# google-deepmind/meltingpot

Measured on NVIDIA H100. Metric: env_steps_per_sec, higher is better.
Workload: dtype u8

## Files before the change

include/mp_engine.h:

```cpp
#ifndef MP_ENGINE_H_
#define MP_ENGINE_H_

#include <stddef.h>
#include <stdint.h>

#ifdef __cplusplus
extern "C" {
#endif

typedef struct mp_engine* mp_handle;

enum {
  MP_OK = 0,
  MP_E_INVALID = -1,
  MP_E_UNSUPPORTED = -2,
  MP_E_CUDA = -3,
  MP_E_NO_DEVICE = -4
};

enum {
  MP_FLAG_RENDER_WORLD = 1u << 0,
  MP_FLAG_RENDER_PLAYERS = 1u << 1,
  MP_FLAG_DEFAULT = 3u,
  MP_FLAG_DEBUG_NO_COMPOSE = 1u << 4,
  MP_FLAG_DEBUG_NO_STORE = 1u << 5,
  MP_FLAG_DEBUG_REUSE_RECORDS = 1u << 6,
  MP_FLAG_DEBUG_NO_FENCE = 1u << 7,
  MP_FLAG_DEBUG_TOP_SPRITE_ONLY = 1u << 8,
  MP_FLAG_DEBUG_PLAIN_LANE_MAP = 1u << 9,
  MP_FLAG_DEBUG_SCATTER_LANE_MAP = 1u << 10,
  MP_FLAG_DEBUG_NO_PREMERGE = 1u << 11,
  MP_FLAG_LAYOUT_TEAMS_SHIFT = 16,
  MP_FLAG_LAYOUT_WARPS_SHIFT = 19,
  MP_FLAG_LAYOUT_WLOG_SHIFT = 24,
  MP_FLAG_LAYOUT_MASK = 0x3ffu << 16
};
#define MP_RENDER_LAYOUT(teams, warps, wlog) \
  (((uint32_t)(teams) << MP_FLAG_LAYOUT_TEAMS_SHIFT) | ((uint32_t)(warps) << MP_FLAG_LAYOUT_WARPS_SHIFT) | ((uint32_t)(wlog) << MP_FLAG_LAYOUT_WLOG_SHIFT))
#define MP_FLAGS_CREATE_ONLY (MP_FLAG_DEBUG_PLAIN_LANE_MAP | MP_FLAG_DEBUG_SCATTER_LANE_MAP | MP_FLAG_DEBUG_NO_PREMERGE | MP_FLAG_LAYOUT_MASK)

typedef struct mp_buffers {
  int32_t num_envs, num_players;
  int32_t rgb_h, rgb_w;
  int32_t world_h, world_w;
  int32_t num_actions;
  int32_t num_scalar_obs;
  uint8_t* rgb;
  uint8_t* world_rgb;
  double* reward;
  double* discount;
  int64_t* step_type;
  double* scalar_obs;
  int32_t* avatar_state;
  uint16_t* grid;
  int32_t grid_layers, grid_cells, grid_cells_padded;
  double* timestep_packed;
  int32_t* events;
  int32_t* event_count;
  int32_t max_events;
// ... 81 lines not shown
```

meltingpot_b200/csrc/engine.cu:

```cuda
#include <cuda_runtime.h>

#include <algorithm>
#include <cstdio>
#include <cstring>
#include <string>
#include <vector>

#include "../../include/mp_engine.h"
#include "../../include/mpb_format.h"
#include "common.cuh"
#include "family_load.h"
#include "render.cuh"
#include "step_clean_up.cuh"
#include "step_commons.cuh"
#include "step_territory.cuh"
#include "step_coins.cuh"
#include "step_mining.cuh"

namespace {

constexpr int kRenderSmemLimit = 227 * 1024 - 2560;
constexpr int kMaxAtlasSprites = 96;
#define MP_MAX_DEVICES 64
#define MP_EXCHANGE_HEADER 256
// ... 406 lines not shown
  for (int i = 0; i < n_total; ++i)
    for (int px = 0; px < 256; ++px) { const uint8_t a = img[(size_t)i * 1024 + px * 4 + 3]; if (a != 0 && a != 255) { binary_alpha[i] = 0; break; } }
  for (int i = 0; i < n_total; ++i) {
    bool bin = true;
    for (int v = 0; v <= T.P; ++v) bin = bin && binary_alpha[smap[(size_t)v * n_total + i]];
    bool invisible = true;
    for (int v = 0; v <= T.P && invisible; ++v) {
      const int t = smap[(size_t)v * n_total + i];
      for (int px = 0; px < 256 && invisible; ++px) invisible = img[(size_t)t * 1024 + px * 4 + 3] == 0;
    }
    sflags[i] = (uint8_t)((opq[i] ? 1 : 0) | (remapped[i] ? 2 : 0) | (bin ? 4 : 0) | (invisible ? 8 : 0));
  }
  E->host_pair = pair; E->host_sflags = sflags;
  E->black_sprite = -1;
  for (int i = 0; i < n_total && E->black_sprite < 0; ++i) {
    if (!opq[i] || remapped[i]) continue;
    bool black = true;
    for (int px = 0; px < 256 && black; ++px) { const uint8_t* q = &img[(size_t)i * 1024 + px * 4]; black = q[0] == 0 && q[1] == 0 && q[2] == 0; }
    if (black) E->black_sprite = i;
  }
  if ((rc = upload(E->allocs, smap, &T.sprite_map)) || (rc = upload(E->allocs, sflags, &T.sprite_opaque)) || (rc = upload(E->allocs, pair, &T.sprite_pair))) return rc;
  return MP_OK;
}

int build_plan(mp_engine* E) {
  const Tables& T = E->T;
  RenderPlan& R = E->R;
  R.view_w = T.view_l + T.view_r + 1; R.view_h = T.view_f + T.view_b + 1;
  R.player_bytes = R.view_w * R.view_h * 192;
  R.world_bytes = T.H * T.W * 192;
  R.grid_bytes = T.L * T.cells_pad * 2;
  R.n_total = E->n_total;
  R.atlas_bytes = R.n_total * 1024;
  R.rec_stride = (int)round_up(T.L + 1, 4);
  R.magic_view_h = (65536u + R.view_h - 1) / R.view_h;
  int off = 128;
  R.off_atlas = off; off += round_up(R.atlas_bytes, 128);
  R.off_pair = off; off += round_up(R.n_total * R.n_total, 128);
  R.off_map = off; off += round_up((T.P + 1) * R.n_total * 2, 128);
  R.off_team0 = off;
  const int f_teams = (E->flags >> MP_FLAG_LAYOUT_TEAMS_SHIFT) & 7, f_warps = (E->flags >> MP_FLAG_LAYOUT_WARPS_SHIFT) & 31,
            f_wlog = (E->flags >> MP_FLAG_LAYOUT_WLOG_SHIFT) & 3;
  const bool forced = (E->flags & MP_FLAG_LAYOUT_MASK) != 0;
  if (forced) {
    if (f_teams < 2 || f_teams > RENDER_MAX_TEAMS || f_warps < 4 || f_warps > TEAM_THREADS / 32 || f_wlog < 1 || f_wlog > 2)
      return fail(MP_E_INVALID, "render layout (%d teams, %d warps, wstrip_log2 %d) outside 2-%d / 4-%d / 1-2", f_teams, f_warps, f_wlog,
                  RENDER_MAX_TEAMS, TEAM_THREADS / 32);
    if (f_teams * f_warps > RENDER_MAX_THREADS / 32)
      return fail(MP_E_UNSUPPORTED, "render layout of %d teams x %d warps exceeds %d threads per CTA", f_teams, f_warps, RENDER_MAX_THREADS);
  }
  R.smem_bytes = 1 << 30;
  int need_forced = 0;
  double best = -1.0;
  for (int teams = 2; teams <= RENDER_MAX_TEAMS; ++teams)
    for (int warps = TEAM_THREADS / 32; warps >= 4; --warps) {
      if (teams * warps > RENDER_MAX_THREADS / 32) continue;
      if (forced && (teams != f_teams || warps != f_warps)) continue;
      for (int wlog = 2; wlog >= 1; --wlog) {
        if (forced && wlog != f_wlog) continue;
        const int stage = RENDER_SLOTS * round_up(std::max(R.view_w * 192, T.W * 24 * (1 << wlog)), 128);
        const int team_bytes = round_up(R.grid_bytes, 128) + round_up(T.cells * R.rec_stride * 2, 128) + warps * stage;
        const int total = R.off_team0 + teams * team_bytes;
        if (forced) need_forced = total;
        if (total > kRenderSmemLimit) continue;
        const double items = T.P * R.view_h + (8 >> wlog) * T.H, per_warp = items / warps;
        const double score = std::min(teams * warps, 18) * per_warp / (per_warp + 4.0) * (wlog == 2 ? 1.0 : 0.85) * (1.0 + 0.1 * teams);
        if (score > best + 1e-9) {
          best = score;
          R.n_teams = teams; R.team_threads = warps * 32; R.wstrip_log2 = wlog; R.stage_bytes = stage;
          R.toff_grid = 0; R.toff_rec = round_up(R.grid_bytes, 128);
          R.toff_stage = R.toff_rec + round_up(T.cells * R.rec_stride * 2, 128);
          R.team_stride = team_bytes; R.smem_bytes = total;
        }
      }
    }
  if (forced && R.smem_bytes > kRenderSmemLimit)
    return fail(MP_E_UNSUPPORTED, "render layout (%d teams, %d warps, wstrip_log2 %d) needs %d B of shared memory (> %d)", f_teams, f_warps,
                f_wlog, need_forced, kRenderSmemLimit);
  if (R.smem_bytes > kRenderSmemLimit) return fail(MP_E_UNSUPPORTED, "render kernel needs %d B of shared memory (> 227 KB)", R.smem_bytes);
  return MP_OK;
}

__global__ void k_debug_obs(Tables T, State S, int32_t* position, int32_t* orientation, int32_t* layer, int32_t* zap, int view_w, int view_h) {
  const int b = blockIdx.x, P = T.P;
  const int32_t* av = S.avatar + (size_t)b * P * 4;
  for (int p = threadIdx.x; p < P; p += blockDim.x) {
    if (position) { position[((size_t)b * P + p) * 2] = av[p * 4 + AV_X]; position[((size_t)b * P + p) * 2 + 1] = av[p * 4 + AV_Y]; }
    if (orientation) orientation[(size_t)b * P + p] = av[p * 4 + AV_ORIENT];
  }
  if (layer) {
    const int per_player = view_h * view_w * T.L;
    const uint16_t* grid = S.grid + (size_t)b * T.L * T.cells_pad;
    for (int i = threadIdx.x; i < P * per_player; i += blockDim.x) {
      const int p = i / per_player, r = i - p * per_player, l = r % T.L, c = r / T.L, vx = c % view_w, vy = c / view_w;
      int x = av[p * 4 + AV_X] - T.view_l + vx, y = av[p * 4 + AV_Y] - T.view_f + vy;
      int32_t v = -1;
      if (wrap_or_reject(T, x, y)) { const uint16_t g = grid[(size_t)l * T.cells_pad + y * T.W + x]; v = g ? ((g - 1) >> 2) + 1 : 0; }
      layer[(size_t)b * P * per_player + i] = v;
    }
  }
  if (zap) {
    for (int i = threadIdx.x; i < P * P; i += blockDim.x) zap[(size_t)b * P * P + i] = 0;
    __syncthreads();
    const int n = min(S.n_events[b], S.max_events);
// ... 535 lines not shown
  memcpy(&hd, host_src, sizeof(hd));
  if (memcmp(hd.magic, "MPS3", 4) != 0 || hd.version != 3u) return fail(MP_E_INVALID, "mp_state_load: not a snapshot (or one of an older engine)");
  if (hd.num_envs != (uint64_t)h->B || hd.payload_bytes != h->state_bytes || hd.n_spans != h->state_spans.size())
    return fail(MP_E_INVALID, "mp_state_load: snapshot of %llu envs / %llu bytes does not fit this engine (%d envs / %llu bytes)",
                (unsigned long long)hd.num_envs, (unsigned long long)hd.payload_bytes, h->B, (unsigned long long)h->state_bytes);
  if (nbytes != sizeof(SnapshotHeader) + hd.payload_bytes)
    return fail(MP_E_INVALID, "mp_state_load: buffer of %llu bytes, snapshot needs %llu (truncated?)", (unsigned long long)nbytes,
                (unsigned long long)(sizeof(SnapshotHeader) + hd.payload_bytes));
  if (hd.blob_hash != h->blob_hash) return fail(MP_E_INVALID, "mp_state_load: snapshot was taken from a different compiled substrate");
  if (hd.rng_key0 != h->S.seed) return fail(MP_E_INVALID, "mp_state_load: snapshot was taken with a different seed / env_index_base (key %llu, engine %llu)",
                                            (unsigned long long)hd.rng_key0, (unsigned long long)h->S.seed);
  DeviceGuard guard(h->device);
  cudaStream_t st = (cudaStream_t)stream;
  const uint8_t* src = static_cast<const uint8_t*>(host_src) + sizeof(hd);
  for (const auto& sp : h->state_spans) {
    CUDA_TRY(cudaMemcpyAsync(sp.first, src, sp.second, cudaMemcpyHostToDevice, st));
    src += sp.second;
  }
  int rc = launch_render(h, st);
  if (rc) return rc;
  CUDA_TRY(cudaStreamSynchronize(st));
  return MP_OK;
}

int mp_launch_count(mp_handle h, uint64_t* out) {
  if (!h || !out) return fail(MP_E_INVALID, "null argument");
  *out = h->launches;
  return MP_OK;
}

int mp_debug_render_plan(mp_handle h, int32_t out[MP_RENDER_PLAN_FIELDS]) {
  if (!h || !out) return fail(MP_E_INVALID, "mp_debug_render_plan: null argument");
  const RenderPlan& R = h->R;
  const int32_t v[MP_RENDER_PLAN_FIELDS] = {R.n_teams, R.team_threads, R.wstrip_log2, R.smem_bytes, R.n_total, R.rec_stride, R.stage_bytes,
                                            R.grid_bytes, h->lane_map_players, h->lane_map_world, h->inst_ncp, h->inst_ncw};
  memcpy(out, v, sizeof v);
  return MP_OK;
}

int mp_debug_render_tables(mp_handle h, int32_t* n_total, uint8_t* pair, uint8_t* flags) {
  if (!h) return fail(MP_E_INVALID, "null handle");
  if (n_total) *n_total = h->n_total;
  if (pair) memcpy(pair, h->host_pair.data(), h->host_pair.size());
  if (flags) memcpy(flags, h->host_sflags.data(), h->host_sflags.size());
  return MP_OK;
}

int mp_debug_observations(mp_handle h, int32_t* position, int32_t* orientation, int32_t* layer, int32_t* zap_matrix, void* stream) {
  if (!h) return fail(MP_E_INVALID, "null handle");
  DeviceGuard guard(h->device);
  k_debug_obs<<<h->B, 128, 0, (cudaStream_t)stream>>>(h->T, h->S, position, orientation, layer, zap_matrix, h->R.view_w, h->R.view_h);
  ++h->launches;
  CUDA_TRY(cudaGetLastError());
  return MP_OK;
}

int mp_debug_lane_map(int n_rows, int n_cells, int pitch_slots, int iters, int scattered, uint32_t out[32]) {
  if (!out || (n_rows != 8 && n_rows != 4 && n_rows != 2) || n_cells < 1 || n_cells > 62 || iters < 1 || iters > 5) return fail(MP_E_INVALID, "mp_debug_lane_map: bad arguments");
  if (!scattered) { if (n_cells > (32 / n_rows) * iters) return fail(MP_E_INVALID, "mp_debug_lane_map: too few turns"); make_lane_map_cells(n_rows, n_cells, pitch_slots, iters, out); return MP_OK; }
  if (!make_lane_map(n_rows, n_cells, pitch_slots, iters, out)) return fail(MP_E_UNSUPPORTED, "no conflict-free dealing for %d rows x %d cells in %d turns", n_rows, n_cells, iters);
  return MP_OK;
}

int mp_algorithmic_bytes(mp_handle h, uint64_t* per_env_step, uint64_t* render_per_env_step) {
  if (!h) return fail(MP_E_INVALID, "null handle");
  if (per_env_step) *per_env_step = h->algo_bytes;
  if (render_per_env_step) *render_per_env_step = h->render_bytes;
// ... 5 lines not shown
```

meltingpot_b200/csrc/render.cuh:

```cuda
#pragma once

#include <cstdio>

#include "common.cuh"

#define RENDER_MAX_TEAMS 4
#define RENDER_MAX_THREADS 1024
#ifndef TEAM_THREADS
#define TEAM_THREADS 512
#endif
#ifndef RENDER_SLOTS
#define RENDER_SLOTS 1
#endif

struct RenderPlan {
  int view_w, view_h;
  int player_bytes;
  int world_bytes;
  int grid_bytes;
  int atlas_bytes;
  int n_total;
  int rec_stride;
  uint32_t magic_view_h;
  int off_atlas, off_pair, off_map, off_team0, team_stride;
  int toff_grid, toff_rec, toff_stage;
  int wstrip_log2;
  int stage_bytes;
  int smem_bytes;
  int team_threads;
  int n_teams;
  int n_player_items, n_items;
  int prow_bytes, wrow_bytes;
  int pitem_bytes, witem_bytes;
  int h_oob, h_oov;
  int h_empty;
  uint32_t pmap[32], wmap[32];
};

__device__ __forceinline__ uint32_t smem_u32(const void* p) { return (uint32_t)__cvta_generic_to_shared(p); }

__device__ __forceinline__ void mbar_init(uint64_t* bar, int count) {
  asm volatile("mbarrier.init.shared::cta.b64 [%0], %1;" ::"r"(smem_u32(bar)), "r"(count));
}
__device__ __forceinline__ void mbar_expect_tx(uint64_t* bar, uint32_t bytes) {
  asm volatile("mbarrier.arrive.expect_tx.shared::cta.b64 _, [%0], %1;" ::"r"(smem_u32(bar)), "r"(bytes) : "memory");
}
__device__ __forceinline__ void mbar_wait(uint64_t* bar, uint32_t parity) {
  asm volatile(
      "{\n"
      ".reg .pred p;\n"
      "WAIT_%=:\n"
      "mbarrier.try_wait.parity.shared::cta.b64 p, [%0], %1;\n"
      "@p bra DONE_%=;\n"
      "bra WAIT_%=;\n"
      "DONE_%=:\n"
      "}\n" ::"r"(smem_u32(bar)), "r"(parity) : "memory");
}
__device__ __forceinline__ void bulk_load(void* dst_smem, const void* src_gmem, uint32_t bytes, uint64_t* bar) {
// ... 7 lines not shown
  return policy;
}
__device__ __forceinline__ void bulk_store(void* dst_gmem, const void* src_smem, uint32_t bytes, uint64_t policy) {
  asm volatile("cp.async.bulk.global.shared::cta.bulk_group.L2::cache_hint [%0], [%1], %2, %3;" ::"l"(dst_gmem), "r"(smem_u32(src_smem)),
               "r"(bytes), "l"(policy)
               : "memory");
  asm volatile("cp.async.bulk.commit_group;" ::: "memory");
}
template <int N>
__device__ __forceinline__ void bulk_wait_read() {
  asm volatile("cp.async.bulk.wait_group.read %0;" ::"n"(N) : "memory");
}
__device__ __forceinline__ void fence_async_smem() { asm volatile("fence.proxy.async.shared::cta;" ::: "memory"); }
__device__ __forceinline__ void group_sync(int bar_id, int threads) { asm volatile("bar.sync %0, %1;" ::"r"(bar_id), "r"(threads) : "memory"); }

__device__ __forceinline__ uint32_t blend_px(uint32_t dst, uint32_t src) {
  const uint32_t a = src >> 24;
  const uint32_t ia = 255u - a;
  uint32_t rb = (src & 0x00FF00FFu) * a + (dst & 0x00FF00FFu) * ia;
  uint32_t g = ((src >> 8) & 0xFFu) * a + ((dst >> 8) & 0xFFu) * ia;
  rb += 0x00010001u; rb += (rb >> 8) & 0x00FF00FFu; rb = (rb >> 8) & 0x00FF00FFu;
  g += 1u; g += g >> 8; g = (g >> 8) & 0xFFu;
  return rb | (g << 8);
}

#define ENT_SHIFT 13
#define ENT_VALUE 0x1fff
#define ENT_OPAQUE 0x2000
#define ENT_REMAP 0x4000
#define ENT_BINARY 0x8000

__device__ __forceinline__ uint32_t select_px(uint32_t dst, uint32_t src) { return (int32_t)src < 0 ? src : dst; }

__device__ __forceinline__ void compose_row(uint32_t px[8], const uint8_t* __restrict__ s_atlas, const uint16_t* __restrict__ rec,
                                            const int16_t* __restrict__ s_map, int viewer_orient, int py) {
  const int n = rec[0];
#pragma unroll
  for (int k = 0; k < 8; ++k) px[k] = 0;
  for (int k = 1; k <= n; ++k) {
    const uint32_t e = rec[k];
    int sprite = (e & ENT_VALUE) >> 2;
    if (e & ENT_REMAP) sprite = s_map[sprite];
    const int facing = ((int)(e & 3) - viewer_orient) & 3;
    const uint8_t* t = s_atlas + (sprite * 4 + facing) * 256 + py * 16;
    const uint4 lo = *reinterpret_cast<const uint4*>(t);
    const uint4 hi = *reinterpret_cast<const uint4*>(t + 128);
    if (e & ENT_BINARY) {
      px[0] = select_px(px[0], lo.x); px[1] = select_px(px[1], lo.y); px[2] = select_px(px[2], lo.z); px[3] = select_px(px[3], lo.w);
      px[4] = select_px(px[4], hi.x); px[5] = select_px(px[5], hi.y); px[6] = select_px(px[6], hi.z); px[7] = select_px(px[7], hi.w);
    } else {
      px[0] = blend_px(px[0], lo.x); px[1] = blend_px(px[1], lo.y); px[2] = blend_px(px[2], lo.z); px[3] = blend_px(px[3], lo.w);
      px[4] = blend_px(px[4], hi.x); px[5] = blend_px(px[5], hi.y); px[6] = blend_px(px[6], hi.z); px[7] = blend_px(px[7], hi.w);
    }
  }
}

#define REC_FAST 0x8000

template <int LMAX>
__device__ __forceinline__ void cell_pass(const Tables& T, const RenderPlan& R, const uint16_t* __restrict__ s_grid, uint16_t* __restrict__ s_rec,
                                          const uint8_t* __restrict__ s_flags, const uint8_t* __restrict__ s_pair, int gtid, int gthreads, uint32_t dbg) {
  for (int c = gtid; c < T.cells; c += gthreads) {
    uint32_t v[LMAX];
#pragma unroll
    for (int l = 0; l < LMAX; ++l) v[l] = l < T.L ? s_grid[l * T.cells_pad + c] : 0u;
    uint32_t nz = 0, oq = 0;
#pragma unroll
    for (int l = 0; l < LMAX; ++l) {
      const uint32_t f = v[l] ? s_flags[(v[l] - 1) >> 2] : 8u;
      nz |= ((f & 8u) ? 0u : 1u) << l;
      oq |= (f & 1u) << l;
    }
    oq &= ~1u;
    const int lo = oq ? 31 - __clz(oq) : 0;
    uint32_t cand = nz & (0xffffffffu << lo);
    uint16_t* r = s_rec + c * R.rec_stride;
    int n = 0;
    uint32_t cur = 0, cf = 0;
    bool merging = true;
    while (cand) {
      const int l = __ffs(cand) - 1;
      cand &= cand - 1;
      const uint32_t vl = s_grid[l * T.cells_pad + c];
      if (cur == 0) { cur = vl; cf = s_flags[(vl - 1) >> 2]; continue; }
      if (merging) {
        const uint32_t m = s_pair[((cur - 1) >> 2) * R.n_total + ((vl - 1) >> 2)];
        if (m && (((cur - 1) ^ (vl - 1)) & 3u) == 0) { cur = 1 + m * 4 + ((vl - 1) & 3u); cf = 5; continue; }
        merging = false;
      }
      r[1 + n++] = (uint16_t)((cur - 1) | (cf << ENT_SHIFT));
      cur = vl; cf = s_flags[(vl - 1) >> 2];
    }
    if (cur) r[1 + n++] = (uint16_t)((cur - 1) | (cf << ENT_SHIFT));
    if ((n == 1 && (cf & 1u)) || ((dbg & 256u) && cur)) r[0] = (uint16_t)(REC_FAST | (cur - 1));
    else r[0] = n ? (uint16_t)n : (uint16_t)R.h_empty;
  }
}

__device__ __forceinline__ void store_row(uint8_t* dst, const uint32_t px[8]) {
  uint2 a, b, c;
  a.x = __byte_perm(px[0], px[1], 0x4210); a.y = __byte_perm(px[1], px[2], 0x5421);
  b.x = __byte_perm(px[2], px[3], 0x6542); b.y = __byte_perm(px[4], px[5], 0x4210);
  c.x = __byte_perm(px[5], px[6], 0x5421); c.y = __byte_perm(px[6], px[7], 0x6542);
  uint2* d = reinterpret_cast<uint2*>(dst);
  d[0] = a; d[1] = b; d[2] = c;
}

__device__ __forceinline__ void fast_row(uint32_t px[8], const uint8_t* __restrict__ s_atlas, int h, int py) {
  const uint8_t* t = s_atlas + (h & 0x7fff) * 256 + py * 16;
  const uint4 lo = *reinterpret_cast<const uint4*>(t);
  const uint4 hi = *reinterpret_cast<const uint4*>(t + 128);
  px[0] = lo.x; px[1] = lo.y; px[2] = lo.z; px[3] = lo.w; px[4] = hi.x; px[5] = hi.y; px[6] = hi.z; px[7] = hi.w;
}

struct ViewerInfo {
  int ax, ay, ao, alive, fdx, fdy, rdx, rdy;
};

template <int NCP, int NCW, bool GATHER>
__global__ void __launch_bounds__(RENDER_MAX_THREADS, 1) k_render(Tables T, State S, RenderPlan R, uint32_t flags) {
  extern __shared__ __align__(128) uint8_t smem[];
  uint64_t* bar = reinterpret_cast<uint64_t*>(smem);
  uint8_t* s_atlas = smem + R.off_atlas;
  const uint8_t* s_pair = smem + R.off_pair;
  int16_t* s_map = reinterpret_cast<int16_t*>(smem + R.off_map);
  __shared__ uint8_t s_opaque[256];
  __shared__ ViewerInfo s_view_all[RENDER_MAX_TEAMS][MP_MAX_PLAYERS];
  __shared__ int s_next_item[RENDER_MAX_TEAMS];

  const int tid = threadIdx.x;
  int team = 0;
#pragma unroll
  for (int k = 1; k < RENDER_MAX_TEAMS; ++k) team += tid >= k * R.team_threads;
  asm volatile("" : "+r"(team));
  const int ttid = tid - team * R.team_threads;
  const int lane = tid & 31, twarp = ttid >> 5;
  uint8_t* s_team = smem + R.off_team0 + team * R.team_stride;
  uint16_t* s_grid = reinterpret_cast<uint16_t*>(s_team + R.toff_grid);
  uint16_t* s_rec = reinterpret_cast<uint16_t*>(s_team + R.toff_rec);
  uint8_t* s_stage = s_team + R.toff_stage + twarp * R.stage_bytes;
  ViewerInfo* s_view = s_view_all[team];
  uint64_t* gbar = &bar[1 + team];

  const int n_streams = gridDim.x * R.n_teams;
  const int rounds = S.B / n_streams;
  const int tail0 = rounds * n_streams;
  const int n_tail = (S.B - tail0 - (int)blockIdx.x + (int)gridDim.x - 1) / (int)gridDim.x;
  const int n_iters = rounds + (n_tail > 0 ? n_tail : 0);
  const int first = blockIdx.x * R.n_teams + team;
  if (tid == 0) {
    for (int i = 0; i < 1 + R.n_teams; ++i) mbar_init(&bar[i], 1);
    asm volatile("fence.mbarrier_init.release.cluster;" ::: "memory");
  }
  if (ttid == 0) s_next_item[team] = 0;
  asm volatile("griddepcontrol.launch_dependents;" ::: "memory");
  __syncthreads();
  if (tid == 0) {
    mbar_expect_tx(&bar[0], (uint32_t)R.atlas_bytes);
    bulk_load(s_atlas, T.atlas, (uint32_t)R.atlas_bytes, &bar[0]);
  }
  for (int i = tid; i < (T.P + 1) * R.n_total; i += (int)blockDim.x) s_map[i] = T.sprite_map[i];
  for (int i = tid; i < R.n_total; i += (int)blockDim.x) s_opaque[i] = T.sprite_opaque[i];
  for (int i = tid; i < R.n_total * R.n_total; i += (int)blockDim.x) smem[R.off_pair + i] = T.sprite_pair[i];
  asm volatile("griddepcontrol.wait;" ::: "memory");
  if (GATHER && tid == 64 && S.g_step > 1ull) {
    for (int r = 0; r < S.g_world; ++r)
      while (*(const volatile unsigned long long*)(S.g_flags + r) + 1ull < S.g_step) __nanosleep(200);
  }
  if (ttid == 0 && rounds > 0) {
    mbar_expect_tx(gbar, (uint32_t)R.grid_bytes);
    bulk_load(s_grid, S.grid + (size_t)first * T.L * T.cells_pad, (uint32_t)R.grid_bytes, gbar);
  }
  __syncthreads();
  mbar_wait(&bar[0], 0);

  const int wlog = R.wstrip_log2, wrows = 1 << wlog;
  const int slot_bytes = R.stage_bytes / RENDER_SLOTS;
  const uint64_t store_policy = make_evict_first_policy();
  uint32_t pcells = R.pmap[lane], wcells = R.wmap[lane];
  asm volatile("" : "+r"(pcells), "+r"(wcells));
  uint32_t slot = 0;
  int gtid = ttid, gthreads = R.team_threads, bar_id = 1 + team;
  int* next_ctr = &s_next_item[team];
  for (int it = 0; it < n_iters; ++it) {
    if (it == rounds) {
      __syncthreads();
      uint8_t* s_team0 = smem + R.off_team0;
      s_grid = reinterpret_cast<uint16_t*>(s_team0 + R.toff_grid);
      s_rec = reinterpret_cast<uint16_t*>(s_team0 + R.toff_rec);
      s_view = s_view_all[0];
      gbar = &bar[1];
      next_ctr = &s_next_item[0];
      gtid = tid; gthreads = (int)blockDim.x; bar_id = 0;
      if (tid == 0) {
        mbar_expect_tx(gbar, (uint32_t)R.grid_bytes);
        bulk_load(s_grid, S.grid + (size_t)(tail0 + (int)blockIdx.x) * T.L * T.cells_pad, (uint32_t)R.grid_bytes, gbar);
      }
    }
    const int b = it < rounds ? first + it * n_streams : tail0 + (int)blockIdx.x + (it - rounds) * (int)gridDim.x;
    if (gtid < T.P) {
      const int4 a = *reinterpret_cast<const int4*>(S.avatar + ((size_t)b * T.P + gtid) * 4);
      ViewerInfo vi;
      vi.ax = a.x; vi.ay = a.y; vi.ao = a.z; vi.alive = a.w;
      vi.fdx = dir_dx(a.z); vi.fdy = dir_dy(a.z); vi.rdx = dir_dx((a.z + 1) & 3); vi.rdy = dir_dy((a.z + 1) & 3);
      s_view[gtid] = vi;
    }
    mbar_wait(gbar, (uint32_t)(it & 1));
    if (!(flags & 64u) || it == 0) {
      if (T.L <= 8) cell_pass<8>(T, R, s_grid, s_rec, s_opaque, s_pair, gtid, gthreads, flags);
      else if (T.L <= 10) cell_pass<10>(T, R, s_grid, s_rec, s_opaque, s_pair, gtid, gthreads, flags);
      else if (T.L <= 12) cell_pass<12>(T, R, s_grid, s_rec, s_opaque, s_pair, gtid, gthreads, flags);
      else cell_pass<MP_MAX_LAYERS>(T, R, s_grid, s_rec, s_opaque, s_pair, gtid, gthreads, flags);
    }
    group_sync(bar_id, gthreads);
    if (gtid == 0 && it + 1 < n_iters && it + 1 != rounds) {
      const int nb = it + 1 < rounds ? b + n_streams : b + (int)gridDim.x;
      mbar_expect_tx(gbar, (uint32_t)R.grid_bytes);
      bulk_load(s_grid, S.grid + (size_t)nb * T.L * T.cells_pad, (uint32_t)R.grid_bytes, gbar);
    }

    int next_item = 0;
    if (lane == 0) next_item = atomicAdd(next_ctr, 1);
    for (;;) {
      const int item = __shfl_sync(MP_FULL, next_item, 0);
      if (item >= R.n_items) break;
      if (lane == 0) next_item = atomicAdd(next_ctr, 1);
      uint8_t* buf = s_stage + (slot % RENDER_SLOTS) * slot_bytes;
      ++slot;
      if (lane == 0) bulk_wait_read<RENDER_SLOTS - 1>();
      __syncwarp();
      if (item < R.n_player_items) {
        const int p = (int)(((uint32_t)item * R.magic_view_h) >> 16), cy = item - p * R.view_h;
        const ViewerInfo vi = s_view[p];
        const int16_t* map = s_map + p * R.n_total;
        const int py = lane & 7;
        const int df = T.view_f - cy;
        const int bx = vi.ax + vi.fdx * df - vi.rdx * T.view_l, by = vi.ay + vi.fdy * df - vi.rdy * T.view_l;
        int hdr[NCP];
        if (!(flags & 16u)) {
        int myh = R.h_oov;
        if (lane < R.view_w && vi.alive) {
          int wx = bx + vi.rdx * lane, wy = by + vi.rdy * lane;
          if (wrap_or_reject(T, wx, wy)) {
            const int cell = wy * T.W + wx, h = s_rec[cell * R.rec_stride];
            myh = (h & REC_FAST) ? ((h & ~3) | ((h - vi.ao) & 3)) : cell;
          } else {
            myh = R.h_oob;
          }
        }
#pragma unroll
        for (int i = 0; i < NCP; ++i) hdr[i] = __shfl_sync(MP_FULL, myh, (pcells >> (6 * i)) & 31);
#pragma unroll
        for (int i = 0; i < NCP; ++i) {
          const int cx = (pcells >> (6 * i)) & 63;
          uint32_t q[8];
          fast_row(q, s_atlas, (hdr[i] & REC_FAST) ? hdr[i] : 0, py);
          if (!(hdr[i] & REC_FAST)) compose_row(q, s_atlas, s_rec + hdr[i] * R.rec_stride, map, vi.ao, py);
          if (cx < R.view_w) store_row(buf + py * R.prow_bytes + cx * 24, q);
        }
        }
        if (!(flags & 128u)) fence_async_smem();
        __syncwarp();
        if (lane == 0 && !(flags & 32u)) {
          const size_t off = ((size_t)b * T.P + p) * R.player_bytes + (size_t)cy * R.pitem_bytes;
          bulk_store(S.rgb + off, buf, (uint32_t)R.pitem_bytes, store_policy);
          if (GATHER) for (int r = 0; r < S.g_world; ++r) bulk_store(S.g_rgb[r] + off, buf, (uint32_t)R.pitem_bytes, store_policy);
        }
      } else {
        const int wi = item - R.n_player_items, wy = wi >> (3 - wlog);
        const int py = ((wi & ((8 >> wlog) - 1)) << wlog) | (lane & (wrows - 1));
        const int16_t* map = s_map + T.P * R.n_total;
        const uint16_t* rowrec = s_rec + wy * T.W * R.rec_stride;
        int hdr[NCW];
        if (!(flags & 16u)) {
#pragma unroll
        for (int i = 0; i < NCW; ++i) {
          const int cx = (wcells >> (6 * i)) & 63;
          hdr[i] = cx < T.W ? (int)rowrec[cx * R.rec_stride] : R.h_oov;
        }
#pragma unroll
        for (int i = 0; i < NCW; ++i) {
          const int cx = (wcells >> (6 * i)) & 63;
          uint32_t q[8];
          fast_row(q, s_atlas, (hdr[i] & REC_FAST) ? hdr[i] : 0, py);
          if (!(hdr[i] & REC_FAST)) compose_row(q, s_atlas, rowrec + min(cx, T.W - 1) * R.rec_stride, map, 0, py);
          if (cx < T.W) store_row(buf + (py & (wrows - 1)) * R.wrow_bytes + cx * 24, q);
        }
        }
        if (!(flags & 128u)) fence_async_smem();
        __syncwarp();
        if (lane == 0 && !(flags & 32u)) {
          const size_t off = (size_t)b * R.world_bytes + (size_t)wi * R.witem_bytes;
          bulk_store(S.world_rgb + off, buf, (uint32_t)R.witem_bytes, store_policy);
          if (GATHER) for (int r = 0; r < S.g_world; ++r) bulk_store(S.g_wrgb[r] + off, buf, (uint32_t)R.witem_bytes, store_policy);
        }
      }
    }
    if (S.x_raise && it == 0) exchange_push(T, S);
    group_sync(bar_id, gthreads);
    if (gtid == 0) *next_ctr = 0;
  }
  if (lane == 0) { if (GATHER) asm volatile("cp.async.bulk.wait_group 0;" ::: "memory"); else bulk_wait_read<0>(); }
}
```

meltingpot_b200/engine.py:

```python

from __future__ import annotations

import ctypes
import os
from typing import Dict, Optional

import numpy as np

_HERE = os.path.dirname(os.path.abspath(__file__))
LIB_PATH = os.environ.get('MP_ENGINE_LIB') or os.path.join(_HERE, 'libmpengine.so')

MP_FLAG_RENDER_WORLD = 1
MP_FLAG_RENDER_PLAYERS = 2
MP_FLAG_DEFAULT = 3
MP_FLAG_DEBUG_PLAIN_LANE_MAP = 1 << 9
MP_FLAG_DEBUG_SCATTER_LANE_MAP = 1 << 10
MP_FLAG_DEBUG_NO_PREMERGE = 1 << 11
MP_FLAG_LAYOUT_MASK = 0x3ff << 16
LANE_MAP_PLAIN, LANE_MAP_SCATTER = 0, 2

RENDER_LAYOUT_RANGES = ((2, 4), (4, 16), (1, 2))


def pack_render_layout(teams: int, warps: int, wstrip_log2: int) -> int:
# ... 369 lines not shown
    out = {'POSITION': torch.empty((B, P, 2), dtype=torch.int32, device=dev),
           'ORIENTATION': torch.empty((B, P), dtype=torch.int32, device=dev)}
    if layer:
      out['LAYER'] = torch.empty((B, P, b.rgb_h // 8, b.rgb_w // 8, b.grid_layers), dtype=torch.int32, device=dev)
    if zap_matrix:
      out['ZAP_MATRIX'] = torch.empty((B, P, P), dtype=torch.int32, device=dev)
    ptr = lambda k: ctypes.c_void_p(out[k].data_ptr()) if k in out else None
    _check(self._lib.mp_debug_observations(self._h, ptr('POSITION'), ptr('ORIENTATION'), ptr('LAYER'), ptr('ZAP_MATRIX'),
                                           self._stream(stream)))
    return out

  def reset_host(self, outputs, stream=None) -> None:
    s = self._host_struct(outputs)
    _check(self._lib.mp_reset_host(self._h, ctypes.byref(s), self._stream(stream)))

  def launch_count(self) -> int:
    n = ctypes.c_uint64(0)
    _check(self._lib.mp_launch_count(self._h, ctypes.byref(n)))
    return int(n.value)

  def save_state(self, stream=None) -> bytes:
    n = ctypes.c_uint64(0)
    _check(self._lib.mp_state_size(self._h, ctypes.byref(n)))
    buf = ctypes.create_string_buffer(n.value)
    _check(self._lib.mp_state_save(self._h, buf, self._stream(stream)))
    return buf.raw

  def load_state(self, snapshot: bytes, stream=None) -> None:
    snapshot = bytes(snapshot)
    buf = ctypes.create_string_buffer(snapshot, len(snapshot))
    _check(self._lib.mp_state_load(self._h, buf, ctypes.c_uint64(len(snapshot)), self._stream(stream)))

  def render_plan(self):
    keys = ('teams', 'team_threads', 'wstrip_log2', 'smem_bytes', 'atlas_sprites', 'rec_stride', 'stage_bytes', 'grid_bytes',
            'lane_map_players', 'lane_map_world', 'ncp', 'ncw')
    out = (ctypes.c_int32 * len(keys))()
    _check(self._lib.mp_debug_render_plan(self._h, out))
    return dict(zip(keys, (int(v) for v in out)))

  def render_tables(self):
    import numpy as np
    n = ctypes.c_int32(0)
    _check(self._lib.mp_debug_render_tables(self._h, ctypes.byref(n), None, None))
    pair = np.zeros((n.value, n.value), np.uint8)
    flags = np.zeros((n.value,), np.uint8)
    _check(self._lib.mp_debug_render_tables(self._h, ctypes.byref(n), pair.ctypes.data, flags.ctypes.data))
    return pair, flags

  def algorithmic_bytes(self):
    a, r = ctypes.c_uint64(0), ctypes.c_uint64(0)
    _check(self._lib.mp_algorithmic_bytes(self._h, ctypes.byref(a), ctypes.byref(r)))
    return int(a.value), int(r.value)


def ipc_export(device_ptr: int):
  handle = ctypes.create_string_buffer(64)
  off = ctypes.c_uint64(0)
  _check(load_library().mp_ipc_export(ctypes.c_void_p(int(device_ptr)), handle, ctypes.byref(off)))
  return handle.raw, int(off.value)


def ipc_open(device: int, handle: bytes, offset: int) -> int:
  ptr = ctypes.c_void_p()
  buf = ctypes.create_string_buffer(bytes(handle), 64)
  _check(load_library().mp_ipc_open(int(device), buf, ctypes.c_uint64(int(offset)), ctypes.byref(ptr)))
  return int(ptr.value)

# ... 4 lines not shown
```

Baseline: 8.935 million.

## Double-buffer render grid in place and drop per-cell record arrays

Replaces the per-cell record array with a compact header array. The merged sprite stack is now written back in place into the grid columns in shared memory. The freed shared memory goes to double-buffering the grid and headers per team, so the next env's grid bulk load can be issued right after the header pass and the trailing group sync per iteration is removed. Viewer info is stored as raw int4 with the direction vectors recomputed per item, and the REUSE_RECORDS debug flag is removed. The risks are extra mbarriers, parity bookkeeping across the tail phase, and the rendered grid being overwritten while the async load for the other slot is in flight.

Result: no change. 8.941 million, median of 6 (+0.1%).

```diff
diff --git a/include/mp_engine.h b/include/mp_engine.h
--- a/include/mp_engine.h
+++ b/include/mp_engine.h
@@ -24,7 +24,6 @@
   MP_FLAG_DEFAULT = 3u,
   MP_FLAG_DEBUG_NO_COMPOSE = 1u << 4,
   MP_FLAG_DEBUG_NO_STORE = 1u << 5,
-  MP_FLAG_DEBUG_REUSE_RECORDS = 1u << 6,
   MP_FLAG_DEBUG_NO_FENCE = 1u << 7,
   MP_FLAG_DEBUG_TOP_SPRITE_ONLY = 1u << 8,
   MP_FLAG_DEBUG_PLAIN_LANE_MAP = 1u << 9,
diff --git a/meltingpot_b200/csrc/engine.cu b/meltingpot_b200/csrc/engine.cu
--- a/meltingpot_b200/csrc/engine.cu
+++ b/meltingpot_b200/csrc/engine.cu
@@ -462,9 +462,13 @@
   R.grid_bytes = T.L * T.cells_pad * 2;
   R.n_total = E->n_total;
   R.atlas_bytes = R.n_total * 1024;
-  R.rec_stride = (int)round_up(T.L + 1, 4);
   R.magic_view_h = (65536u + R.view_h - 1) / R.view_h;
+  R.grid_pitch = (int)round_up(R.grid_bytes, 16);
+  R.hdr_stride = (int)round_up(T.cells, 8);
+  R.toff_grid = 0; R.toff_hdr = 2 * R.grid_pitch;
+  R.toff_stage = R.toff_hdr + 2 * R.hdr_stride * 2;
   int off = 128;
+  static_assert(8 * (1 + 2 * RENDER_MAX_TEAMS) <= 128, "render mbarriers outgrow their block");
   R.off_atlas = off; off += round_up(R.atlas_bytes, 128);
   R.off_pair = off; off += round_up(R.n_total * R.n_total, 128);
   R.off_map = off; off += round_up((T.P + 1) * R.n_total * 2, 128);
@@ -489,7 +493,7 @@
       for (int wlog = 2; wlog >= 1; --wlog) {
         if (forced && wlog != f_wlog) continue;
         const int stage = RENDER_SLOTS * round_up(std::max(R.view_w * 192, T.W * 24 * (1 << wlog)), 128);
-        const int team_bytes = round_up(R.grid_bytes, 128) + round_up(T.cells * R.rec_stride * 2, 128) + warps * stage;
+        const int team_bytes = R.toff_stage + warps * stage;
         const int total = R.off_team0 + teams * team_bytes;
         if (forced) need_forced = total;
         if (total > kRenderSmemLimit) continue;
@@ -498,8 +502,6 @@
         if (score > best + 1e-9) {
           best = score;
           R.n_teams = teams; R.team_threads = warps * 32; R.wstrip_log2 = wlog; R.stage_bytes = stage;
-          R.toff_grid = 0; R.toff_rec = round_up(R.grid_bytes, 128);
-          R.toff_stage = R.toff_rec + round_up(T.cells * R.rec_stride * 2, 128);
           R.team_stride = team_bytes; R.smem_bytes = total;
         }
       }
@@ -1101,7 +1103,7 @@
 int mp_debug_render_plan(mp_handle h, int32_t out[MP_RENDER_PLAN_FIELDS]) {
   if (!h || !out) return fail(MP_E_INVALID, "mp_debug_render_plan: null argument");
   const RenderPlan& R = h->R;
-  const int32_t v[MP_RENDER_PLAN_FIELDS] = {R.n_teams, R.team_threads, R.wstrip_log2, R.smem_bytes, R.n_total, R.rec_stride, R.stage_bytes,
+  const int32_t v[MP_RENDER_PLAN_FIELDS] = {R.n_teams, R.team_threads, R.wstrip_log2, R.smem_bytes, R.n_total, R.hdr_stride, R.stage_bytes,
                                             R.grid_bytes, h->lane_map_players, h->lane_map_world, h->inst_ncp, h->inst_ncw};
   memcpy(out, v, sizeof v);
   return MP_OK;
diff --git a/meltingpot_b200/csrc/render.cuh b/meltingpot_b200/csrc/render.cuh
--- a/meltingpot_b200/csrc/render.cuh
+++ b/meltingpot_b200/csrc/render.cuh
@@ -20,10 +20,10 @@
   int grid_bytes;
   int atlas_bytes;
   int n_total;
-  int rec_stride;
+  int hdr_stride;
   uint32_t magic_view_h;
   int off_atlas, off_pair, off_map, off_team0, team_stride;
-  int toff_grid, toff_rec, toff_stage;
+  int toff_grid, grid_pitch, toff_hdr, toff_stage;
   int wstrip_log2;
   int stage_bytes;
   int smem_bytes;
@@ -97,69 +97,83 @@
 
 __device__ __forceinline__ uint32_t select_px(uint32_t dst, uint32_t src) { return (int32_t)src < 0 ? src : dst; }
 
-__device__ __forceinline__ void compose_row(uint32_t px[8], const uint8_t* __restrict__ s_atlas, const uint16_t* __restrict__ rec,
-                                            const int16_t* __restrict__ s_map, int viewer_orient, int py) {
-  const int n = rec[0];
-#pragma unroll
-  for (int k = 0; k < 8; ++k) px[k] = 0;
-  for (int k = 1; k <= n; ++k) {
-    const uint32_t e = rec[k];
-    int sprite = (e & ENT_VALUE) >> 2;
-    if (e & ENT_REMAP) sprite = s_map[sprite];
-    const int facing = ((int)(e & 3) - viewer_orient) & 3;
-    const uint8_t* t = s_atlas + (sprite * 4 + facing) * 256 + py * 16;
-    const uint4 lo = *reinterpret_cast<const uint4*>(t);
-    const uint4 hi = *reinterpret_cast<const uint4*>(t + 128);
-    if (e & ENT_BINARY) {
-      px[0] = select_px(px[0], lo.x); px[1] = select_px(px[1], lo.y); px[2] = select_px(px[2], lo.z); px[3] = select_px(px[3], lo.w);
-      px[4] = select_px(px[4], hi.x); px[5] = select_px(px[5], hi.y); px[6] = select_px(px[6], hi.z); px[7] = select_px(px[7], hi.w);
-    } else {
-      px[0] = blend_px(px[0], lo.x); px[1] = blend_px(px[1], lo.y); px[2] = blend_px(px[2], lo.z); px[3] = blend_px(px[3], lo.w);
-      px[4] = blend_px(px[4], hi.x); px[5] = blend_px(px[5], hi.y); px[6] = blend_px(px[6], hi.z); px[7] = blend_px(px[7], hi.w);
+__device__ __forceinline__ void compose_entry(uint32_t px[8], uint32_t e, const uint8_t* __restrict__ s_atlas, const int16_t* __restrict__ s_map,
+                                              int viewer_orient, int py) {
+  int sprite = (e & ENT_VALUE) >> 2;
+  if (e & ENT_REMAP) sprite = s_map[sprite];
+  const int facing = ((int)(e & 3) - viewer_orient) & 3;
+  const uint8_t* t = s_atlas + (sprite * 4 + facing) * 256 + py * 16;
+  const uint4 lo = *reinterpret_cast<const uint4*>(t);
+  const uint4 hi = *reinterpret_cast<const uint4*>(t + 128);
+  if (e & ENT_BINARY) {
+    px[0] = select_px(px[0], lo.x); px[1] = select_px(px[1], lo.y); px[2] = select_px(px[2], lo.z); px[3] = select_px(px[3], lo.w);
+    px[4] = select_px(px[4], hi.x); px[5] = select_px(px[5], hi.y); px[6] = select_px(px[6], hi.z); px[7] = select_px(px[7], hi.w);
+  } else {
+    px[0] = blend_px(px[0], lo.x); px[1] = blend_px(px[1], lo.y); px[2] = blend_px(px[2], lo.z); px[3] = blend_px(px[3], lo.w);
+    px[4] = blend_px(px[4], hi.x); px[5] = blend_px(px[5], hi.y); px[6] = blend_px(px[6], hi.z); px[7] = blend_px(px[7], hi.w);
+  }
+}
+
+#define REC_FAST 0x8000
+
+__device__ __forceinline__ void layer_bits(uint32_t v, int l, const uint8_t* __restrict__ s_flags, uint32_t& nz, uint32_t& oq) {
+  const uint32_t f = v ? s_flags[(v - 1) >> 2] : 8u;
+  nz |= ((f & 8u) ? 0u : 1u) << l;
+  oq |= (f & 1u) << l;
+}
+
+__device__ __forceinline__ uint32_t stack_candidates(uint32_t nz, uint32_t oq) {
+  oq &= ~1u;
+  const int lo = oq ? 31 - __clz(oq) : 0;
+  return nz & (0xffffffffu << lo);
+}
+
+template <typename Emit>
+__device__ __forceinline__ void walk_stack(uint32_t cand, const uint16_t* g, int cells_pad, const uint8_t* __restrict__ s_flags,
+                                           const uint8_t* __restrict__ s_pair, int n_total, Emit&& emit) {
+  uint32_t cur = 0, cf = 0;
+  bool merging = true;
+  while (cand) {
+    const int l = __ffs(cand) - 1;
+    cand &= cand - 1;
+    const uint32_t vl = g[l * cells_pad];
+    if (cur == 0) { cur = vl; cf = s_flags[(vl - 1) >> 2]; continue; }
+    if (merging) {
+      const uint32_t m = s_pair[((cur - 1) >> 2) * n_total + ((vl - 1) >> 2)];
+      if (m && (((cur - 1) ^ (vl - 1)) & 3u) == 0) { cur = 1 + m * 4 + ((vl - 1) & 3u); cf = 5; continue; }
+      merging = false;
     }
-  }
-}
-
-#define REC_FAST 0x8000
+    emit((cur - 1) | (cf << ENT_SHIFT));
+    cur = vl; cf = s_flags[(vl - 1) >> 2];
+  }
+  if (cur) emit((cur - 1) | (cf << ENT_SHIFT));
+}
 
 template <int LMAX>
-__device__ __forceinline__ void cell_pass(const Tables& T, const RenderPlan& R, const uint16_t* __restrict__ s_grid, uint16_t* __restrict__ s_rec,
-                                          const uint8_t* __restrict__ s_flags, const uint8_t* __restrict__ s_pair, int gtid, int gthreads, uint32_t dbg) {
+__device__ __forceinline__ void header_pass(const Tables& T, const RenderPlan& R, uint16_t* s_grid, uint16_t* __restrict__ s_hdr,
+                                            const uint8_t* __restrict__ s_flags, const uint8_t* __restrict__ s_pair, int gtid, int gthreads, uint32_t dbg) {
   for (int c = gtid; c < T.cells; c += gthreads) {
     uint32_t v[LMAX];
 #pragma unroll
     for (int l = 0; l < LMAX; ++l) v[l] = l < T.L ? s_grid[l * T.cells_pad + c] : 0u;
     uint32_t nz = 0, oq = 0;
 #pragma unroll
-    for (int l = 0; l < LMAX; ++l) {
-      const uint32_t f = v[l] ? s_flags[(v[l] - 1) >> 2] : 8u;
-      nz |= ((f & 8u) ? 0u : 1u) << l;
-      oq |= (f & 1u) << l;
-    }
-    oq &= ~1u;
-    const int lo = oq ? 31 - __clz(oq) : 0;
-    uint32_t cand = nz & (0xffffffffu << lo);
-    uint16_t* r = s_rec + c * R.rec_stride;
+    for (int l = 0; l < LMAX; ++l) layer_bits(v[l], l, s_flags, nz, oq);
+    const uint32_t cand = stack_candidates(nz, oq);
     int n = 0;
-    uint32_t cur = 0, cf = 0;
-    bool merging = true;
-    while (cand) {
-      const int l = __ffs(cand) - 1;
-      cand &= cand - 1;
-      const uint32_t vl = s_grid[l * T.cells_pad + c];
-      if (cur == 0) { cur = vl; cf = s_flags[(vl - 1) >> 2]; continue; }
-      if (merging) {
-        const uint32_t m = s_pair[((cur - 1) >> 2) * R.n_total + ((vl - 1) >> 2)];
-        if (m && (((cur - 1) ^ (vl - 1)) & 3u) == 0) { cur = 1 + m * 4 + ((vl - 1) & 3u); cf = 5; continue; }
-        merging = false;
-      }
-      r[1 + n++] = (uint16_t)((cur - 1) | (cf << ENT_SHIFT));
-      cur = vl; cf = s_flags[(vl - 1) >> 2];
-    }
-    if (cur) r[1 + n++] = (uint16_t)((cur - 1) | (cf << ENT_SHIFT));
-    if ((n == 1 && (cf & 1u)) || ((dbg & 256u) && cur)) r[0] = (uint16_t)(REC_FAST | (cur - 1));
-    else r[0] = n ? (uint16_t)n : (uint16_t)R.h_empty;
-  }
+    uint32_t last = 0;
+    uint16_t* col = s_grid + c;
+    walk_stack(cand, col, T.cells_pad, s_flags, s_pair, R.n_total, [&](uint32_t e) { col[n * T.cells_pad] = (uint16_t)e; ++n; last = e; });
+    const bool fast = (n == 1 && (last & ENT_OPAQUE)) || ((dbg & 256u) && n);
+    s_hdr[c] = (uint16_t)(fast ? (REC_FAST | (last & ENT_VALUE)) : n ? n : R.h_empty);
+  }
+}
+
+__device__ __forceinline__ void compose_cell(uint32_t px[8], int cells_pad, int n, const uint16_t* __restrict__ g,
+                                             const uint8_t* __restrict__ s_atlas, const int16_t* __restrict__ s_map, int viewer_orient, int py) {
+#pragma unroll
+  for (int k = 0; k < 8; ++k) px[k] = 0;
+  for (int k = 0; k < n; ++k) compose_entry(px, g[k * cells_pad], s_atlas, s_map, viewer_orient, py);
 }
 
 __device__ __forceinline__ void store_row(uint8_t* dst, const uint32_t px[8]) {
@@ -177,10 +191,6 @@
   const uint4 hi = *reinterpret_cast<const uint4*>(t + 128);
   px[0] = lo.x; px[1] = lo.y; px[2] = lo.z; px[3] = lo.w; px[4] = hi.x; px[5] = hi.y; px[6] = hi.z; px[7] = hi.w;
 }
-
-struct ViewerInfo {
-  int ax, ay, ao, alive, fdx, fdy, rdx, rdy;
-};
 
 template <int NCP, int NCW, bool GATHER>
 __global__ void __launch_bounds__(RENDER_MAX_THREADS, 1) k_render(Tables T, State S, RenderPlan R, uint32_t flags) {
@@ -190,8 +200,8 @@
   const uint8_t* s_pair = smem + R.off_pair;
   int16_t* s_map = reinterpret_cast<int16_t*>(smem + R.off_map);
   __shared__ uint8_t s_opaque[256];
-  __shared__ ViewerInfo s_view_all[RENDER_MAX_TEAMS][MP_MAX_PLAYERS];
-  __shared__ int s_next_item[RENDER_MAX_TEAMS];
+  __shared__ int4 s_view_all[RENDER_MAX_TEAMS][2][MP_MAX_PLAYERS];
+  __shared__ int s_next_item[RENDER_MAX_TEAMS][2];
 
   const int tid = threadIdx.x;
   int team = 0;
@@ -200,12 +210,8 @@
   asm volatile("" : "+r"(team));
   const int ttid = tid - team * R.team_threads;
   const int lane = tid & 31, twarp = ttid >> 5;
-  uint8_t* s_team = smem + R.off_team0 + team * R.team_stride;
-  uint16_t* s_grid = reinterpret_cast<uint16_t*>(s_team + R.toff_grid);
-  uint16_t* s_rec = reinterpret_cast<uint16_t*>(s_team + R.toff_rec);
-  uint8_t* s_stage = s_team + R.toff_stage + twarp * R.stage_bytes;
-  ViewerInfo* s_view = s_view_all[team];
-  uint64_t* gbar = &bar[1 + team];
+  uint8_t* s_stage = smem + R.off_team0 + team * R.team_stride + R.toff_stage + twarp * R.stage_bytes;
+  int gteam = team;
 
   const int n_streams = gridDim.x * R.n_teams;
   const int rounds = S.B / n_streams;
@@ -213,11 +219,12 @@
   const int n_tail = (S.B - tail0 - (int)blockIdx.x + (int)gridDim.x - 1) / (int)gridDim.x;
   const int n_iters = rounds + (n_tail > 0 ? n_tail : 0);
   const int first = blockIdx.x * R.n_teams + team;
+  auto grid_of = [&](int t, int slot) { return reinterpret_cast<uint16_t*>(smem + R.off_team0 + t * R.team_stride + R.toff_grid + slot * R.grid_pitch); };
   if (tid == 0) {
-    for (int i = 0; i < 1 + R.n_teams; ++i) mbar_init(&bar[i], 1);
+    for (int i = 0; i < 1 + 2 * R.n_teams; ++i) mbar_init(&bar[i], 1);
     asm volatile("fence.mbarrier_init.release.cluster;" ::: "memory");
   }
-  if (ttid == 0) s_next_item[team] = 0;
+  if (ttid < 2) s_next_item[team][ttid] = 0;
   asm volatile("griddepcontrol.launch_dependents;" ::: "memory");
   __syncthreads();
   if (tid == 0) {
@@ -233,57 +240,52 @@
       while (*(const volatile unsigned long long*)(S.g_flags + r) + 1ull < S.g_step) __nanosleep(200);
   }
   if (ttid == 0 && rounds > 0) {
-    mbar_expect_tx(gbar, (uint32_t)R.grid_bytes);
-    bulk_load(s_grid, S.grid + (size_t)first * T.L * T.cells_pad, (uint32_t)R.grid_bytes, gbar);
+    mbar_expect_tx(&bar[1 + 2 * team], (uint32_t)R.grid_bytes);
+    bulk_load(grid_of(team, 0), S.grid + (size_t)first * T.L * T.cells_pad, (uint32_t)R.grid_bytes, &bar[1 + 2 * team]);
   }
   __syncthreads();
   mbar_wait(&bar[0], 0);
 
   const int wlog = R.wstrip_log2, wrows = 1 << wlog;
   const int slot_bytes = R.stage_bytes / RENDER_SLOTS;
-  const uint64_t store_policy = make_evict_first_policy();
   uint32_t pcells = R.pmap[lane], wcells = R.wmap[lane];
   asm volatile("" : "+r"(pcells), "+r"(wcells));
   uint32_t slot = 0;
   int gtid = ttid, gthreads = R.team_threads, bar_id = 1 + team;
-  int* next_ctr = &s_next_item[team];
   for (int it = 0; it < n_iters; ++it) {
     if (it == rounds) {
       __syncthreads();
-      uint8_t* s_team0 = smem + R.off_team0;
-      s_grid = reinterpret_cast<uint16_t*>(s_team0 + R.toff_grid);
-      s_rec = reinterpret_cast<uint16_t*>(s_team0 + R.toff_rec);
-      s_view = s_view_all[0];
-      gbar = &bar[1];
-      next_ctr = &s_next_item[0];
+      gteam = 0;
       gtid = tid; gthreads = (int)blockDim.x; bar_id = 0;
       if (tid == 0) {
-        mbar_expect_tx(gbar, (uint32_t)R.grid_bytes);
-        bulk_load(s_grid, S.grid + (size_t)(tail0 + (int)blockIdx.x) * T.L * T.cells_pad, (uint32_t)R.grid_bytes, gbar);
+        mbar_expect_tx(&bar[1 + (rounds & 1)], (uint32_t)R.grid_bytes);
+        bulk_load(grid_of(0, rounds & 1), S.grid + (size_t)(tail0 + (int)blockIdx.x) * T.L * T.cells_pad, (uint32_t)R.grid_bytes,
+                  &bar[1 + (rounds & 1)]);
       }
     }
+    const int s = it & 1;
     const int b = it < rounds ? first + it * n_streams : tail0 + (int)blockIdx.x + (it - rounds) * (int)gridDim.x;
-    if (gtid < T.P) {
-      const int4 a = *reinterpret_cast<const int4*>(S.avatar + ((size_t)b * T.P + gtid) * 4);
-      ViewerInfo vi;
-      vi.ax = a.x; vi.ay = a.y; vi.ao = a.z; vi.alive = a.w;
-      vi.fdx = dir_dx(a.z); vi.fdy = dir_dy(a.z); vi.rdx = dir_dx((a.z + 1) & 3); vi.rdy = dir_dy((a.z + 1) & 3);
-      s_view[gtid] = vi;
+    uint8_t* g_team = smem + R.off_team0 + gteam * R.team_stride;
+    uint16_t* s_grid = reinterpret_cast<uint16_t*>(g_team + R.toff_grid + s * R.grid_pitch);
+    uint16_t* s_hdr = reinterpret_cast<uint16_t*>(g_team + R.toff_hdr) + s * R.hdr_stride;
+    if (gtid < T.P) s_view_all[gteam][s][gtid] = *reinterpret_cast<const int4*>(S.avatar + ((size_t)b * T.P + gtid) * 4);
+    mbar_wait(&bar[1 + 2 * gteam + s], (uint32_t)((it >> 1) & 1));
+    if (T.L <= 8) header_pass<8>(T, R, s_grid, s_hdr, s_opaque, s_pair, gtid, gthreads, flags);
+    else if (T.L <= 10) header_pass<10>(T, R, s_grid, s_hdr, s_opaque, s_pair, gtid, gthreads, flags);
+    else if (T.L <= 12) header_pass<12>(T, R, s_grid, s_hdr, s_opaque, s_pair, gtid, gthreads, flags);
+    else header_pass<MP_MAX_LAYERS>(T, R, s_grid, s_hdr, s_opaque, s_pair, gtid, gthreads, flags);
+    group_sync(bar_id, gthreads);
+    if (gtid == 0) {
+      s_next_item[gteam][s ^ 1] = 0;
+      if (it + 1 < n_iters && it + 1 != rounds) {
+        const int nb = it + 1 < rounds ? b + n_streams : b + (int)gridDim.x;
+        mbar_expect_tx(&bar[1 + 2 * gteam + (s ^ 1)], (uint32_t)R.grid_bytes);
+        bulk_load(grid_of(gteam, s ^ 1), S.grid + (size_t)nb * T.L * T.cells_pad, (uint32_t)R.grid_bytes, &bar[1 + 2 * gteam + (s ^ 1)]);
+      }
     }
-    mbar_wait(gbar, (uint32_t)(it & 1));
-    if (!(flags & 64u) || it == 0) {
-      if (T.L <= 8) cell_pass<8>(T, R, s_grid, s_rec, s_opaque, s_pair, gtid, gthreads, flags);
-      else if (T.L <= 10) cell_pass<10>(T, R, s_grid, s_rec, s_opaque, s_pair, gtid, gthreads, flags);
-      else if (T.L <= 12) cell_pass<12>(T, R, s_grid, s_rec, s_opaque, s_pair, gtid, gthreads, flags);
-      else cell_pass<MP_MAX_LAYERS>(T, R, s_grid, s_rec, s_opaque, s_pair, gtid, gthreads, flags);
-    }
-    group_sync(bar_id, gthreads);
-    if (gtid == 0 && it + 1 < n_iters && it + 1 != rounds) {
-      const int nb = it + 1 < rounds ? b + n_streams : b + (int)gridDim.x;
-      mbar_expect_tx(gbar, (uint32_t)R.grid_bytes);
-      bulk_load(s_grid, S.grid + (size_t)nb * T.L * T.cells_pad, (uint32_t)R.grid_bytes, gbar);
-    }
-
+
+    int* next_ctr = &s_next_item[gteam][s];
+    const int4* s_view = s_view_all[gteam][s];
     int next_item = 0;
     if (lane == 0) next_item = atomicAdd(next_ctr, 1);
     for (;;) {
@@ -296,19 +298,20 @@
       __syncwarp();
       if (item < R.n_player_items) {
         const int p = (int)(((uint32_t)item * R.magic_view_h) >> 16), cy = item - p * R.view_h;
-        const ViewerInfo vi = s_view[p];
+        const int4 vi = s_view[p];
+        const int fdx = dir_dx(vi.z), fdy = dir_dy(vi.z), rdx = dir_dx((vi.z + 1) & 3), rdy = dir_dy((vi.z + 1) & 3);
         const int16_t* map = s_map + p * R.n_total;
         const int py = lane & 7;
         const int df = T.view_f - cy;
-        const int bx = vi.ax + vi.fdx * df - vi.rdx * T.view_l, by = vi.ay + vi.fdy * df - vi.rdy * T.view_l;
+        const int bx = vi.x + fdx * df - rdx * T.view_l, by = vi.y + fdy * df - rdy * T.view_l;
         int hdr[NCP];
         if (!(flags & 16u)) {
         int myh = R.h_oov;
-        if (lane < R.view_w && vi.alive) {
-          int wx = bx + vi.rdx * lane, wy = by + vi.rdy * lane;
+        if (lane < R.view_w && vi.w) {
+          int wx = bx + rdx * lane, wy = by + rdy * lane;
           if (wrap_or_reject(T, wx, wy)) {
-            const int cell = wy * T.W + wx, h = s_rec[cell * R.rec_stride];
-            myh = (h & REC_FAST) ? ((h & ~3) | ((h - vi.ao) & 3)) : cell;
+            const int cell = wy * T.W + wx, h = s_hdr[cell];
+            myh = (h & REC_FAST) ? ((h & ~3) | ((h - vi.z) & 3)) : cell;
           } else {
             myh = R.h_oob;
           }
@@ -320,13 +323,14 @@
           const int cx = (pcells >> (6 * i)) & 63;
           uint32_t q[8];
           fast_row(q, s_atlas, (hdr[i] & REC_FAST) ? hdr[i] : 0, py);
-          if (!(hdr[i] & REC_FAST)) compose_row(q, s_atlas, s_rec + hdr[i] * R.rec_stride, map, vi.ao, py);
+          if (!(hdr[i] & REC_FAST)) compose_cell(q, T.cells_pad, s_hdr[hdr[i]], s_grid + hdr[i], s_atlas, map, vi.z, py);
           if (cx < R.view_w) store_row(buf + py * R.prow_bytes + cx * 24, q);
         }
         }
         if (!(flags & 128u)) fence_async_smem();
         __syncwarp();
         if (lane == 0 && !(flags & 32u)) {
+          const uint64_t store_policy = make_evict_first_policy();
           const size_t off = ((size_t)b * T.P + p) * R.player_bytes + (size_t)cy * R.pitem_bytes;
           bulk_store(S.rgb + off, buf, (uint32_t)R.pitem_bytes, store_policy);
           if (GATHER) for (int r = 0; r < S.g_world; ++r) bulk_store(S.g_rgb[r] + off, buf, (uint32_t)R.pitem_bytes, store_policy);
@@ -335,26 +339,22 @@
         const int wi = item - R.n_player_items, wy = wi >> (3 - wlog);
         const int py = ((wi & ((8 >> wlog) - 1)) << wlog) | (lane & (wrows - 1));
         const int16_t* map = s_map + T.P * R.n_total;
-        const uint16_t* rowrec = s_rec + wy * T.W * R.rec_stride;
-        int hdr[NCW];
+        const uint16_t* rowhdr = s_hdr + wy * T.W;
         if (!(flags & 16u)) {
 #pragma unroll
         for (int i = 0; i < NCW; ++i) {
           const int cx = (wcells >> (6 * i)) & 63;
-          hdr[i] = cx < T.W ? (int)rowrec[cx * R.rec_stride] : R.h_oov;
-        }
-#pragma unroll
-        for (int i = 0; i < NCW; ++i) {
-          const int cx = (wcells >> (6 * i)) & 63;
+          const int h = cx < T.W ? (int)rowhdr[cx] : R.h_oov;
           uint32_t q[8];
-          fast_row(q, s_atlas, (hdr[i] & REC_FAST) ? hdr[i] : 0, py);
-          if (!(hdr[i] & REC_FAST)) compose_row(q, s_atlas, rowrec + min(cx, T.W - 1) * R.rec_stride, map, 0, py);
+          fast_row(q, s_atlas, (h & REC_FAST) ? h : 0, py);
+          if (!(h & REC_FAST)) compose_cell(q, T.cells_pad, h, s_grid + wy * T.W + min(cx, T.W - 1), s_atlas, map, 0, py);
           if (cx < T.W) store_row(buf + (py & (wrows - 1)) * R.wrow_bytes + cx * 24, q);
         }
         }
         if (!(flags & 128u)) fence_async_smem();
         __syncwarp();
         if (lane == 0 && !(flags & 32u)) {
+          const uint64_t store_policy = make_evict_first_policy();
           const size_t off = (size_t)b * R.world_bytes + (size_t)wi * R.witem_bytes;
           bulk_store(S.world_rgb + off, buf, (uint32_t)R.witem_bytes, store_policy);
           if (GATHER) for (int r = 0; r < S.g_world; ++r) bulk_store(S.g_wrgb[r] + off, buf, (uint32_t)R.witem_bytes, store_policy);
@@ -362,8 +362,6 @@
       }
     }
     if (S.x_raise && it == 0) exchange_push(T, S);
-    group_sync(bar_id, gthreads);
-    if (gtid == 0) *next_ctr = 0;
   }
   if (lane == 0) { if (GATHER) asm volatile("cp.async.bulk.wait_group 0;" ::: "memory"); else bulk_wait_read<0>(); }
 }
diff --git a/meltingpot_b200/engine.py b/meltingpot_b200/engine.py
--- a/meltingpot_b200/engine.py
+++ b/meltingpot_b200/engine.py
@@ -425,7 +425,7 @@
     _check(self._lib.mp_state_load(self._h, buf, ctypes.c_uint64(len(snapshot)), self._stream(stream)))
 
   def render_plan(self):
-    keys = ('teams', 'team_threads', 'wstrip_log2', 'smem_bytes', 'atlas_sprites', 'rec_stride', 'stage_bytes', 'grid_bytes',
+    keys = ('teams', 'team_threads', 'wstrip_log2', 'smem_bytes', 'atlas_sprites', 'hdr_stride', 'stage_bytes', 'grid_bytes',
             'lane_map_players', 'lane_map_world', 'ncp', 'ncw')
     out = (ctypes.c_int32 * len(keys))()
     _check(self._lib.mp_debug_render_plan(self._h, out))
```
